# yenanjing/mmEgo

Measured on AMD Instinct MI355X. Metric: train frames/sec (Upper+Lower U+L step, B=64/GPU, T=8, 128 pts), higher is better.
Workload: dtype f32; 1 GPU; U+L step (Train_Upper + Train_Lower train_once bodies), B=64/GPU T=8 N=128, fp32, dropout live, two concurrent HIP-graph branches; global_batch=64, seq_len=8, points=128, parallelism=dp1

## Files before the change

include/mmego_hip.h:

```cpp
#ifndef MMEGO_HIP_H
#define MMEGO_HIP_H
#ifdef __cplusplus
extern "C" {
#endif

int mmego_gemm(void* stream, const float* A, long sam, long sak, const float* B, long sbk, long sbn, float* C,
               long scm, long scn, const float* bias, int M, int N, int K, int nbatch, long sAb, long sBb, long sCb,
               int relu, int accumulate, float* splitk_ws, int nsplit, long sBiasb, const float* cmul, float* asum);
typedef struct MmegoGemmDesc {
  const float* A; long sam, sak;
  const float* B; long sbk, sbn;
  float* C; long scm, scn;
  const float* bias;
  int M, N, K, nbatch;
  long sAb, sBb, sCb;
  int relu, accumulate;
  float* splitk_ws; int nsplit;
  long sBiasb;
  const float* cmul; float* asum;
} MmegoGemmDesc;
int mmego_gemm_group(void* stream, int n, const MmegoGemmDesc* descs);

int mmego_colstats_nblk(long rows);
int mmego_bn_train_stats(void* stream, const float* X, long ldx, long rows, int C, const float* gamma,
// ... 40 lines not shown

int mmego_lstm_step(void* stream, int ndir, int Bn, int H, int first, const float* hprev0, const float* hprev1,
                    long hps, const float* whh0, const float* whh1, const float* bhh0, const float* bhh1,
                    const float* xproj0, const float* xproj1, long xs, float* hout0, float* hout1, long hos, float* c0,
                    float* c1, float* gst0, float* gst1, float* cst0, float* cst1);
int mmego_lstm64_forward(void* stream, int B, int T, const float* xproj0, const float* xproj1, long xs,
                         const float* whh0, const float* whh1, const float* bhh0, const float* bhh1, const float* h0_0,
                         const float* h0_1, const float* c0_0, const float* c0_1, float* out, long os, float* hn0,
                         float* hn1, float* cn0, float* cn1,
                         float* gates0, float* gates1, float* cst0, float* cst1, float* hprev0, float* hprev1,
                         float* drop_y, float* drop_mask, float drop_p, const unsigned long long* seed_ctr, int salt);
int mmego_lstm64_backward(void* stream, int B, int T, const float* dout, long dos, const float* gates0,
                          const float* gates1, const float* cst0, const float* cst1, const float* c0_0,
                          const float* c0_1, const float* whh0, const float* whh1, float* dgates0, float* dgates1,
                          long dgs);

typedef struct MmegoLstm64Fwd {
  const float* xproj[2]; long xs;
  const float* whh[2]; const float* bhh[2]; const float* h0[2]; const float* c0[2];
  float* out; long os;
  float* hn[2]; float* cn[2];
  float* gates[2]; float* cst[2]; float* hprev[2];
  int B, T;
  float* drop_y; float* drop_mask; float drop_p; const unsigned long long* seed_ctr; unsigned salt;
} MmegoLstm64Fwd;
typedef struct MmegoLstm64Bwd {
  const float* dout; long dos;
  const float* gates[2]; const float* cst[2]; const float* c0[2]; const float* whh[2];
  float* dgates[2]; long dgs;
  int B, T;
} MmegoLstm64Bwd;
int mmego_lstm64_forward_multi(void* stream, int n, const void* descs);
int mmego_lstm64_backward_multi(void* stream, int n, const void* descs);

int mmego_cvt_bf16(void* stream, const float* X, long ldx, long rows, long cols, unsigned short* Y, long ldy);
int mmego_cvt_bf16_tm(void* stream, const float* X, long ldx, int Bn, int T, long cols, unsigned short* Y, int Bp);
int mmego_gemm_bf16(void* stream, const unsigned short* A, long lda, const unsigned short* W, long ldw, float* C,
                    long ldc, unsigned short* Cb, long ldcb, float* Cf, const float* bias, int M, int N, int K, int relu);
int mmego_lstm_step_bf16(void* stream, int ndir, int Bn, int H, int first, const unsigned short* hprev0,
                         const unsigned short* hprev1, const unsigned short* whh0, const unsigned short* whh1,
                         const float* xpf, long mt0_0, long mt0_1, float* hout0, float* hout1,
                         long hos, unsigned short* houtb0, unsigned short* houtb1, long hbs,
                         unsigned short* hfrag0, unsigned short* hfrag1, float* c0, float* c1);

int mmego_lstm_step_bf16_fused(void* stream, int ndir, int Bn, int H, int first, int nseg,
                               const unsigned short* a0_0, const unsigned short* a0_1, const unsigned short* w0_0,
                               const unsigned short* w0_1, int K0, const unsigned short* a1_0,
                               const unsigned short* a1_1, const unsigned short* w1_0, const unsigned short* w1_1,
                               int K1, const unsigned short* hprev0, const unsigned short* hprev1,
                               const unsigned short* whh0, const unsigned short* whh1, const float* bias,
                               float* hout0, float* hout1, long hos, unsigned short* hfrag0, unsigned short* hfrag1,
                               float* c0, float* c1);
int mmego_attn_pool_frag_bf16_ok(int H);
int mmego_attn_pool_frag_bf16(void* stream, const unsigned short* hf, int T, int Bp, int Bn, int H, const float* w, const float* b,
                              float* vec, float* attn);
int mmego_cvt_bf16_frag_tm(void* stream, const float* X, long ldx, int Bn, int T, int C, unsigned short* Y, int Bp);
int mmego_fc_relu_bf16_frag_tm(void* stream, const float* X, long ldx, const float* W, const float* bias, int Bn, int T, int Cin,
                               int H, unsigned short* Y, int Bp, int relu);

int mmego_lstm_cell_backward(void* stream, int ndir, int Bn, int H, const float* dout0, const float* dout1, long dos,
                             const float* dhrec0, const float* dhrec1, const float* gst0, const float* gst1,
                             const float* cst0, const float* cst1, const float* cprev0, const float* cprev1, float* dc0,
                             float* dc1, float* dgates0, float* dgates1, long dgs);
int mmego_imu_loss(void* stream, const float* R, const float* t, const float* R_gt, const float* head_gt, long F,
                   float scale, float* loss, float* dR, float* dt);
int mmego_lstm_bwd_step(void* stream, int Bn, int H, const float* dg0, const float* dg1, long dgs, const float* wT0,
// ... 238 lines not shown
```

mmego_amd/csrc/gemm.hip:

```cpp
#include <stdlib.h>

#include "common.h"
#include "../../include/mmego_hip.h"

#include "gemm_tile.h"
#include "lstm_cell.h"
#include "tile_order.h"

struct GemmP {
  const float* A;
  const float* B;
  float* C;
  const float* bias;
  long sam, sak, sbk, sbn, scm, scn;
  long sAb, sBb, sCb, sCs, sBiasb;
  int M, N, K;
  int nsplit, kchunk;
  int relu, accumulate;
  int avec, bvec;
  const float* cmul;
  float* asum;
  const float* cb_dout[2]; long cb_dos;
  const float* cb_gst[2]; const float* cb_cst[2]; const float* cb_cprev[2];
  float* cb_dc[2]; float* cb_dg[2]; long cb_dgs;
// ... 415 lines not shown
    const float bv = bias ? bias[col] : 0.0f;
#pragma unroll
    for (int i = 0; i < 2; ++i) {
#pragma unroll
      for (int reg = 0; reg < 16; ++reg) {
        int row = m0 + wm * 64 + i * 32 + (reg & 3) + 8 * (reg >> 2) + 4 * (lane >> 5);
        float v = acc[i][j][reg] + bv;
        if (relu) v = fmaxf(v, 0.0f);
        C[(long)row * ldc + col] = v;
      }
    }
  }
}

extern "C" int mmego_gemm(void* stream, const float* A, long sam, long sak, const float* B, long sbk, long sbn,
                          float* C, long scm, long scn, const float* bias, int M, int N, int K, int nbatch, long sAb,
                          long sBb, long sCb, int relu, int accumulate, float* splitk_ws, int nsplit, long sBiasb,
                          const float* cmul, float* asum) {
  MMEGO_REQUIRE(A && B && C && M > 0 && N > 0 && K > 0 && nbatch > 0 && nsplit >= 1);
  const bool defer = accumulate == 2;
  MMEGO_REQUIRE(!defer || (nsplit > 1 && nbatch == 1 && !bias && !relu));
  MMEGO_REQUIRE(!cmul || nsplit == 1);
  MMEGO_REQUIRE(relu == 0 || relu == 1 || (relu == 2 && cmul));
  MMEGO_REQUIRE(sBiasb == 0 || nsplit == 1);
  hipStream_t st = (hipStream_t)stream;
  {
    const bool a_kc = sak == 1, a_mc = sam == 1 && !a_kc;
    const bool b_kc = sbk == 1, b_mc = sbn == 1 && !b_kc;
    const long lda = a_kc ? sam : sak, ldw = b_kc ? sbn : sbk;
    const int kchunk_t = nsplit > 1 ? cdiv(cdiv(K, nsplit), 64) * 64 : K;
    constexpr long tile_min_other = GEMM_TILE_MIN_OTHER;
    const long tile_min_units = (a_kc && b_kc && nsplit == 1) ? (K <= 1024 ? 1 : 200) : tile_min_other;
    const long units64 = (long)(M / 64) * (N / 64) * nsplit * nbatch;
    const bool ok = !cmul && !asum && scn == 1 && (nbatch == 1 || ((sAb % 4) == 0 && (sBb % 4) == 0)) && (a_kc || a_mc) && (b_kc || b_mc) && (lda % 4) == 0 && (ldw % 4) == 0 &&
                    (((uintptr_t)A | (uintptr_t)B) & 15) == 0 && (M % 64) == 0 && (N % 64) == 0 &&
                    (K % 64) == 0 && units64 >= tile_min_units && (nsplit == 1 || (long)(nsplit - 1) * kchunk_t < K);
    if (ok) {
      TileP tp;
      tp.A = A; tp.W = B; tp.C = C; tp.bias = bias;
      tp.M = M; tp.N = N; tp.K = K;
      tp.lda = lda; tp.ldw = ldw; tp.ldc = scm;
      tp.relu = relu; tp.accumulate = accumulate;
      tp.nsplit = nsplit; tp.kchunk = kchunk_t; tp.ws = splitk_ws;
      tp.nbatch = nbatch; tp.sAb = sAb; tp.sWb = sBb; tp.sCb = sCb; tp.sBiasb = sBiasb;
      int rc = mmego_detail::gemm_tile_launch(st, tp, a_kc, b_kc);
      if (rc == 0 && nsplit > 1 && !defer) {
        long total = (long)nbatch * M * N;
        int blocks = (int)((total + SKR_OUT - 1) / SKR_OUT);
        hipLaunchKernelGGL(splitk_reduce_kernel, dim3(blocks), dim3(256), 0, st, splitk_ws, C, bias, nsplit, nbatch, M, N, scm, scn,
                           sCb, relu, accumulate, (const float*)nullptr, (float*)nullptr);
        MMEGO_LAUNCH_CHECK();
      }
      if (rc != -2) return rc;
    }
  }
  const bool fast = !cmul && !asum && nbatch == 1 && nsplit == 1 && !accumulate && sak == 1 && sbk == 1 && scn == 1 && (M % 128) == 0 &&
                    (N % 128) == 0 && (K % 16) == 0 && (sam % 4) == 0 && (sbn % 4) == 0 &&
                    (((uintptr_t)A | (uintptr_t)B) & 15) == 0;
  if (fast) {
    dim3 grid((M / 128) * (N / 128));
    hipLaunchKernelGGL(gemm128_nt_kernel, grid, dim3(256), 0, st, A, B, C, bias, M, N, K, sam, sbn, scm, relu);
    MMEGO_LAUNCH_CHECK();
    return MMEGO_OK;
  }
  GemmP p;
  p.A = A; p.B = B; p.bias = bias;
  p.sam = sam; p.sak = sak; p.sbk = sbk; p.sbn = sbn;
  p.sAb = sAb; p.sBb = sBb; p.sBiasb = sBiasb;
  p.M = M; p.N = N; p.K = K;
  p.nsplit = nsplit;
  p.relu = relu; p.accumulate = accumulate;
  p.cmul = cmul;
  p.asum = asum;
  p.cb_dg[0] = p.cb_dg[1] = nullptr;
  if (nsplit > 1) {
    MMEGO_REQUIRE(splitk_ws != nullptr);
    int kc = cdiv(K, nsplit);
// ... 131 lines not shown
```

mmego_amd/csrc/gemm_tile.h:

```cpp
#pragma once
#include <hip/hip_runtime.h>

struct TileP {
  const float* A;
  const float* W;
  float* C;
  const float* bias;
  int M, N, K;
  long lda, ldw, ldc;
  int relu, accumulate;
  int nsplit, kchunk;
  float* ws;
  int nbatch;
  long sAb, sWb, sCb, sBiasb;
};

namespace mmego_detail {
int gemm_tile_launch(hipStream_t st, const TileP& p, bool a_kc, bool b_kc);
}
```

mmego_amd/csrc/gemm_tile.hip:

```cpp
#include <stdlib.h>

#include "common.h"
#include "gemm_tile.h"
#include "lds_dma.h"
#include "tile_order.h"

#define TLD_MAX 68

template <int BM, int BN, int WAVES_M, int WAVES_N, bool A_KC, bool B_KC, int KCH>
__device__ __forceinline__ void gemm_tile_body(const TileP& p, int m0, int n0, int sb, float* smem, int sid) {
  const int split = sb % p.nsplit, batch = sb / p.nsplit;
  static_assert(WAVES_M * WAVES_N == 4, "4 waves");
  static_assert(KCH == 64 || KCH == 32, "k per staged chunk");
  constexpr int TLD = KCH + 4;
  constexpr int WM = BM / WAVES_M, WN = BN / WAVES_N;
  constexpr int TM = WM / 32, TN = WN / 32;
  constexpr int AV = BM * KCH / 1024, BV = BN * KCH / 1024;
  constexpr int LPR = KCH / 4, RPP = 256 / LPR;
  constexpr int ALD = BM + 4, BLD = BN + 4;
  constexpr int ARP = 1024 / BM, BRP = 1024 / BN;
  float* As = smem;
  float* Bs = smem + BM * TLD;
  const int tid = threadIdx.x, lane = tid & 63, wave = tid >> 6;
  const int wm = wave % WAVES_M, wn = wave / WAVES_M;
// ... 262 lines not shown
      }
      if (kb == 3) {
        asm volatile("s_waitcnt vmcnt(0) lgkmcnt(0)" ::: "memory");
        __builtin_amdgcn_s_barrier();
        if (kt + 2 < nk) GTB_DMA(kt + 2, kt & 1)
      }
#pragma unroll
      for (int c = 0; c < 4; ++c)
#pragma unroll
        for (int i = 0; i < 5; ++i)
#pragma unroll
          for (int j = 0; j < 2; ++j) acc[i][j] = __builtin_amdgcn_mfma_f32_32x32x2f32(a[i][c], b[j][c], acc[i][j], 0, 0, 0);
    }
  }
#endif
#undef GTB_DMA
  const bool slabs = p.nsplit > 1;
  float* C = slabs ? p.ws + (long)blockIdx.y * p.M * p.N : p.C + (long)batch * p.sCb;
  const long ldc = slabs ? (long)p.N : p.ldc;
#pragma unroll
  for (int j = 0; j < 2; ++j) {
    const int col = n0 + wn * 64 + j * 32 + r;
    const float bv = (p.bias && !slabs) ? p.bias[(long)batch * p.sBiasb + col] : 0.0f;
#pragma unroll
    for (int i = 0; i < 5; ++i) {
      float* cp = C + (long)(m0 + wm * 160 + i * 32 + 4 * h) * ldc + col;
#pragma unroll
      for (int reg = 0; reg < 16; ++reg)
        if (!(GTB_EXP & 4) || acc[i][j][reg] == 12345.f) cp[(long)((reg & 3) + 8 * (reg >> 2)) * ldc] = acc[i][j][reg] + bv;
    }
  }
}

namespace mmego_detail {

constexpr int GT_KCH = 32;

template <int BM, int BN, bool A_KC, bool B_KC, int KCH>
static int launch_plain_k(hipStream_t st, const TileP& p) {
  const size_t lds = (size_t)((BM + BN) * (KCH + 4)) * sizeof(float);
  if (int e = mmego_allow_lds<gemm_tile_kernel<BM, BN, 2, 2, A_KC, B_KC, KCH>>(lds)) return e;
  const unsigned units = (unsigned)((p.M / BM) * (p.N / BN) * p.nsplit * p.nbatch);
  hipLaunchKernelGGL((gemm_tile_kernel<BM, BN, 2, 2, A_KC, B_KC, KCH>), dim3(units), dim3(256), lds, st, p);
  hipError_t e = hipGetLastError();
  return e == hipSuccess ? 0 : (int)e;
}

template <int BM, int BN, bool A_KC, bool B_KC>
static int launch_plain(hipStream_t st, const TileP& p) { return launch_plain_k<BM, BN, A_KC, B_KC, GT_KCH>(st, p); }

template <bool A_KC, bool B_KC>
static int launch_layout(hipStream_t st, const TileP& p) {
  if (A_KC && B_KC) {
    static const bool big = !(getenv("MMEGO_GEMM_BIG") && atoi(getenv("MMEGO_GEMM_BIG")) == 0);
    const long tiles = (long)(p.M / 320) * (p.N / 256) * p.nbatch;
    const bool slab_ok = p.nsplit == 1 ? !p.accumulate
                                       : (p.accumulate == 2 && p.nbatch == 1 && p.ws && !p.bias && (p.kchunk % 32) == 0 && p.kchunk >= 64 &&
                                          (long)(p.nsplit - 1) * p.kchunk < p.K && (p.K - (long)(p.nsplit - 1) * p.kchunk) >= 64);
    const long units = tiles * p.nsplit;
    if (big && (p.M % 320) == 0 && (p.N % 256) == 0 && (p.K % 32) == 0 && p.K >= 64 && slab_ok && !p.relu &&
        units >= 256 && (units % 256) == 0 && tiles < (1L << 30) && (p.lda % 4) == 0 && (p.ldw % 4) == 0 && (p.sAb % 4) == 0 && (p.sWb % 4) == 0 &&
        ((((uintptr_t)p.A) | ((uintptr_t)p.W)) & 15) == 0) {
      constexpr int lds = 2 * (320 + 256) * 32 * (int)sizeof(float);
      if (int e = mmego_allow_lds<gemm_tile_big_kernel<0>>(lds)) return e;
      TileBigArgs g = {p.M / 320, p.N / 256};
      hipLaunchKernelGGL((gemm_tile_big_kernel<0>), dim3((unsigned)tiles, (unsigned)p.nsplit), dim3(512), lds, st, p, g);
      hipError_t e = hipGetLastError();
      return e == hipSuccess ? 0 : (int)e;
    }
  }
  const long units128 = (long)(p.M / 128) * (p.N / 128) * p.nsplit * p.nbatch;
  const bool big_ok = (p.M % 128) == 0 && (p.N % 128) == 0 && units128 >= 192;
  if (big_ok) {
    static const int slots = getenv("MMEGO_GEMM_SLOTS") ? atoi(getenv("MMEGO_GEMM_SLOTS")) : 512;
    const int units = (int)units128;
    if (units > slots && p.K > 128) {
      const int rest = units % slots;
      const bool halves = rest > 0 && rest <= slots / 2;
      const int nfull = halves ? units - rest : units, nhalf = halves ? 2 * rest : 0;
      const size_t lds = slots <= 256 ? 84 * 1024 : (size_t)(256 * (GT_KCH + 4)) * sizeof(float);
      if (int e = mmego_allow_lds<gemm_tile_persistent_kernel<A_KC, B_KC, GT_KCH>>(lds)) return e;
      hipLaunchKernelGGL((gemm_tile_persistent_kernel<A_KC, B_KC, GT_KCH>), dim3(slots), dim3(256), lds, st, p, nfull, nhalf, 1);
      hipError_t e = hipGetLastError();
      return e == hipSuccess ? 0 : (int)e;
    }
    return launch_plain<128, 128, A_KC, B_KC>(st, p);
  }
  return launch_plain<64, 64, A_KC, B_KC>(st, p);
}

int gemm_tile_launch(hipStream_t st, const TileP& p, bool a_kc, bool b_kc) {
  if ((p.K % 64) != 0 || (p.M % 64) != 0 || (p.N % 64) != 0 || p.nsplit < 1 || p.nbatch < 1) return -2;
  if (p.nsplit > 1 && ((p.kchunk % 64) != 0 || p.ws == nullptr)) return -2;
  if (a_kc && b_kc) return launch_layout<true, true>(st, p);
  if (a_kc) return launch_layout<true, false>(st, p);
  if (b_kc) return launch_layout<false, true>(st, p);
  return launch_layout<false, false>(st, p);
}

}
```

mmego_amd/csrc/lstm.hip:

```cpp
#include "common.h"
#include "lstm_cell.h"
#include <stddef.h>
#include "../../include/mmego_hip.h"

struct Lstm64P {
  const float* xproj[2]; long xs;
  const float* whh[2];
  const float* bhh[2];
  const float* h0[2]; const float* c0[2];
  float* out; long os;
  float* hn[2]; float* cn[2];
  float* gates[2]; float* cst[2]; float* hprev[2];
  int B, T;
  float* drop_y; float* drop_mask; float drop_p; const unsigned long long* seed_ctr; unsigned salt;
};


#define L64_LDS_BARRIER() asm volatile("s_waitcnt lgkmcnt(0)\n\ts_barrier" ::: "memory")

#define WLD 272

typedef const float __attribute__((address_space(1)))* l64_gcptr;
typedef float __attribute__((address_space(1)))* l64_gptr;
typedef f32x4 __attribute__((address_space(1)))* l64_gptr4;
// ... 104 lines not shown
          const float mk = dropout_keep(dkey, (unsigned)off, p.drop_p) ? keep_scale : 0.f;
          p.drop_mask[off] = mk;
          p.drop_y[off] = hn * mk;
        }
        if (stash) {
          *(l64_gptr4)gq[reg] = (f32x4){u.i, u.f, u.g, u.o};
          *cq[reg] = cn;
        }
      }
      oq[reg] += ostep;
      if (stash) { gq[reg] += gstep; cq[reg] += cstep; }
    }
    __builtin_amdgcn_sched_barrier(0);
#pragma unroll
    for (int g = 0; g < 4; ++g)
#pragma unroll
      for (int reg = 0; reg < 4; ++reg) xp[g][reg] = xpn[g][reg];
    L64_LDS_BARRIER();
  }
#undef L64_LOAD_XP
#pragma unroll
  for (int reg = 0; reg < 4; ++reg) {
    int row = r0 + fq * 4 + reg;
    if (row < B) {
      if (p.hn[d]) p.hn[d][row * 64 + j] = hreg[reg];
      if (p.cn[d]) p.cn[d][row * 64 + j] = creg[reg];
    }
  }
}

template <bool FULL, bool STASH, bool DROP>
__global__ __launch_bounds__(256) void lstm64_fwd_kernel(Lstm64P p) { lstm64_fwd_body<FULL, STASH, DROP>(p); }

#define L64_MAX_MULTI 4
static_assert(sizeof(Lstm64P) == sizeof(MmegoLstm64Fwd) && offsetof(Lstm64P, seed_ctr) == offsetof(MmegoLstm64Fwd, seed_ctr) &&
              offsetof(Lstm64P, B) == offsetof(MmegoLstm64Fwd, B), "MmegoLstm64Fwd is Lstm64P");
struct Lstm64Multi { Lstm64P p[L64_MAX_MULTI]; };
template <bool FULL, bool STASH, bool DROP>
__global__ __launch_bounds__(256) void lstm64_fwd_multi_kernel(Lstm64Multi m) { lstm64_fwd_body<FULL, STASH, DROP>(m.p[blockIdx.z]); }

extern "C" int mmego_lstm64_forward(void* stream, int B, int T, const float* xproj0, const float* xproj1, long xs,
                                    const float* whh0, const float* whh1, const float* bhh0, const float* bhh1,
                                    const float* h0_0, const float* h0_1, const float* c0_0, const float* c0_1, float* out,
                                    long os, float* hn0, float* hn1,
                                    float* cn0, float* cn1, float* gates0, float* gates1, float* cst0, float* cst1,
                                    float* hprev0, float* hprev1, float* drop_y, float* drop_mask, float drop_p,
                                    const unsigned long long* seed_ctr, int salt) {
  MMEGO_REQUIRE((drop_mask == nullptr) == (drop_y == nullptr));
  MMEGO_REQUIRE(!drop_mask || (seed_ctr && drop_p > 0.f && drop_p < 1.f && (long)B * T * os < (1L << 32)));
  MMEGO_REQUIRE(B > 0 && T > 0 && xproj0 && xproj1 && whh0 && whh1 && out);
  MMEGO_REQUIRE((((uintptr_t)whh0 | (uintptr_t)whh1) & 15) == 0);
  MMEGO_REQUIRE((gates0 == nullptr) == (cst0 == nullptr) && (gates1 == nullptr) == (cst1 == nullptr));
  Lstm64P p;
  p.xproj[0] = xproj0; p.xproj[1] = xproj1; p.xs = xs;
  p.whh[0] = whh0; p.whh[1] = whh1;
  p.bhh[0] = bhh0; p.bhh[1] = bhh1;
  p.h0[0] = h0_0; p.h0[1] = h0_1; p.c0[0] = c0_0; p.c0[1] = c0_1;
  p.out = out; p.os = os;
  p.hn[0] = hn0; p.hn[1] = hn1; p.cn[0] = cn0; p.cn[1] = cn1;
  p.gates[0] = gates0; p.gates[1] = gates1; p.cst[0] = cst0; p.cst[1] = cst1;
  p.hprev[0] = hprev0; p.hprev[1] = hprev1;
  p.B = B; p.T = T;
  p.drop_y = drop_y; p.drop_mask = drop_mask; p.drop_p = drop_p; p.seed_ctr = seed_ctr; p.salt = (unsigned)salt;
  size_t lds = (size_t)(64 * 16) * sizeof(float);
  const bool full = B % 16 == 0, st_ = gates0 != nullptr, dr = drop_mask != nullptr;
  MMEGO_REQUIRE((hprev0 != nullptr) == st_ && (hprev1 != nullptr) == st_ && (gates1 != nullptr) == st_);
#define L64_FWD_LAUNCH(F_, S_, D_)                                                                                    \
  do {                                                                                                                \
    if (int e = mmego_allow_lds<lstm64_fwd_kernel<F_, S_, D_>>(lds)) return e;                                        \
    hipLaunchKernelGGL((lstm64_fwd_kernel<F_, S_, D_>), dim3(cdiv(B, 16), 2), dim3(256), lds, (hipStream_t)stream, p); \
  } while (0)
  if (full) {
    if (st_ && dr) L64_FWD_LAUNCH(true, true, true);
    else if (st_) L64_FWD_LAUNCH(true, true, false);
    else if (dr) L64_FWD_LAUNCH(true, false, true);
    else L64_FWD_LAUNCH(true, false, false);
  } else {
    if (st_ && dr) L64_FWD_LAUNCH(false, true, true);
    else if (st_) L64_FWD_LAUNCH(false, true, false);
    else if (dr) L64_FWD_LAUNCH(false, false, true);
    else L64_FWD_LAUNCH(false, false, false);
  }
#undef L64_FWD_LAUNCH
  MMEGO_LAUNCH_CHECK();
  return MMEGO_OK;
}

struct Lstm64BwdP {
  const float* dout; long dos;
  const float* gates[2]; const float* cst[2]; const float* c0[2];
  const float* whh[2];
  float* dgates[2]; long dgs;
  int B, T;
};


template <bool FULL>
__device__ __forceinline__ void lstm64_bwd_body(const Lstm64BwdP& p) {
  extern __shared__ __attribute__((aligned(16))) float smem[];
  float* dgs = smem;
  const int tid = threadIdx.x, lane = tid & 63, wave = tid >> 6;
// ... 69 lines not shown
#pragma unroll
      for (int g = 0; g < 4; ++g) dgs[(g * 64 + j) * 16 + fq * 4 + reg] = dg4[g][reg];
      ccur[reg] = gin[reg][5];
    }
    L64_LDS_BARRIER();
    f32x4 a0 = {0.f, 0.f, 0.f, 0.f}, a1 = {0.f, 0.f, 0.f, 0.f}, a2 = {0.f, 0.f, 0.f, 0.f}, a3 = {0.f, 0.f, 0.f, 0.f};
#pragma unroll
    for (int nb = 0; nb < 64; nb += 16) {
      float dk[16];
#pragma unroll
      for (int u = 0; u < 16; ++u) dk[u] = dgs[((nb + u) * 4 + fq) * 16 + fr];
      __builtin_amdgcn_sched_barrier(0);
#pragma unroll
      for (int u = 0; u < 16; u += 4) {
        a0 = __builtin_amdgcn_mfma_f32_16x16x4f32(dk[u], wreg[nb + u], a0, 0, 0, 0);
        a1 = __builtin_amdgcn_mfma_f32_16x16x4f32(dk[u + 1], wreg[nb + u + 1], a1, 0, 0, 0);
        a2 = __builtin_amdgcn_mfma_f32_16x16x4f32(dk[u + 2], wreg[nb + u + 2], a2, 0, 0, 0);
        a3 = __builtin_amdgcn_mfma_f32_16x16x4f32(dk[u + 3], wreg[nb + u + 3], a3, 0, 0, 0);
      }
    }
    dhrec = (a0 + a1) + (a2 + a3);
    __builtin_amdgcn_sched_barrier(0);
#pragma unroll
    for (int reg = 0; reg < 4; ++reg)
#pragma unroll
      for (int q = 0; q < 6; ++q) gin[reg][q] = gnx[reg][q];
    L64_LDS_BARRIER();
  }
#undef L64_LOAD_BWD
}

template <bool FULL>
__global__ __launch_bounds__(256) void lstm64_bwd_kernel(Lstm64BwdP p) { lstm64_bwd_body<FULL>(p); }
static_assert(sizeof(Lstm64BwdP) == sizeof(MmegoLstm64Bwd) && offsetof(Lstm64BwdP, dgs) == offsetof(MmegoLstm64Bwd, dgs), "MmegoLstm64Bwd is Lstm64BwdP");
struct Lstm64BwdMulti { Lstm64BwdP p[L64_MAX_MULTI]; };
template <bool FULL>
__global__ __launch_bounds__(256) void lstm64_bwd_multi_kernel(Lstm64BwdMulti m) { lstm64_bwd_body<FULL>(m.p[blockIdx.z]); }

extern "C" int mmego_lstm64_backward(void* stream, int B, int T, const float* dout, long dos, const float* gates0,
                                     const float* gates1, const float* cst0, const float* cst1, const float* c0_0,
                                     const float* c0_1, const float* whh0, const float* whh1, float* dgates0,
                                     float* dgates1, long dgs) {
  MMEGO_REQUIRE(B > 0 && T > 0 && dout && gates0 && gates1 && cst0 && cst1 && whh0 && whh1 && dgates0 && dgates1);
  MMEGO_REQUIRE((((uintptr_t)whh0 | (uintptr_t)whh1) & 15) == 0);
  Lstm64BwdP p;
  p.dout = dout; p.dos = dos;
  p.gates[0] = gates0; p.gates[1] = gates1; p.cst[0] = cst0; p.cst[1] = cst1;
  p.c0[0] = c0_0; p.c0[1] = c0_1;
  p.whh[0] = whh0; p.whh[1] = whh1;
  p.dgates[0] = dgates0; p.dgates[1] = dgates1; p.dgs = dgs;
  p.B = B; p.T = T;
  const size_t lds = (size_t)(256 * 16) * sizeof(float);
  if (B % 16 == 0) hipLaunchKernelGGL(lstm64_bwd_kernel<true>, dim3(cdiv(B, 16), 2), dim3(256), lds, (hipStream_t)stream, p);
  else hipLaunchKernelGGL(lstm64_bwd_kernel<false>, dim3(cdiv(B, 16), 2), dim3(256), lds, (hipStream_t)stream, p);
  MMEGO_LAUNCH_CHECK();
  return MMEGO_OK;
}

extern "C" int mmego_lstm64_forward_multi(void* stream, int n, const void* descs) {
  MMEGO_REQUIRE(descs && n >= 1 && n <= L64_MAX_MULTI);
  const Lstm64P* h = static_cast<const Lstm64P*>(descs);
  Lstm64Multi m;
  const int B = h[0].B, T = h[0].T;
  const bool st_ = h[0].gates[0] != nullptr, dr = h[0].drop_mask != nullptr;
  for (int i = 0; i < n; ++i) {
    const Lstm64P& p = h[i];
    MMEGO_REQUIRE(p.B == B && p.T == T && B > 0 && T > 0 && p.xproj[0] && p.xproj[1] && p.whh[0] && p.whh[1] && p.out);
    MMEGO_REQUIRE((((uintptr_t)p.whh[0] | (uintptr_t)p.whh[1]) & 15) == 0);
    MMEGO_REQUIRE((p.drop_mask == nullptr) == (p.drop_y == nullptr) && (p.drop_mask != nullptr) == dr);
    MMEGO_REQUIRE(!p.drop_mask || (p.seed_ctr && p.drop_p > 0.f && p.drop_p < 1.f && (long)B * T * p.os < (1L << 32)));
    MMEGO_REQUIRE((p.gates[0] != nullptr) == st_ && (p.gates[1] != nullptr) == st_ && (p.cst[0] != nullptr) == st_ && (p.cst[1] != nullptr) == st_ &&
                  (p.hprev[0] != nullptr) == st_ && (p.hprev[1] != nullptr) == st_);
    m.p[i] = p;
  }
  for (int i = n; i < L64_MAX_MULTI; ++i) m.p[i] = h[0];
  const size_t lds = (size_t)(64 * 16) * sizeof(float);
  const bool full = B % 16 == 0;
#define L64_FWDM_LAUNCH(F_, S_, D_) hipLaunchKernelGGL((lstm64_fwd_multi_kernel<F_, S_, D_>), dim3(cdiv(B, 16), 2, n), dim3(256), lds, (hipStream_t)stream, m)
  if (full) {
    if (st_ && dr) L64_FWDM_LAUNCH(true, true, true);
    else if (st_) L64_FWDM_LAUNCH(true, true, false);
    else if (dr) L64_FWDM_LAUNCH(true, false, true);
    else L64_FWDM_LAUNCH(true, false, false);
  } else {
    if (st_ && dr) L64_FWDM_LAUNCH(false, true, true);
    else if (st_) L64_FWDM_LAUNCH(false, true, false);
    else if (dr) L64_FWDM_LAUNCH(false, false, true);
    else L64_FWDM_LAUNCH(false, false, false);
  }
#undef L64_FWDM_LAUNCH
  MMEGO_LAUNCH_CHECK();
  return MMEGO_OK;
}

extern "C" int mmego_lstm64_backward_multi(void* stream, int n, const void* descs) {
  MMEGO_REQUIRE(descs && n >= 1 && n <= L64_MAX_MULTI);
  const Lstm64BwdP* h = static_cast<const Lstm64BwdP*>(descs);
  Lstm64BwdMulti m;
  const int B = h[0].B, T = h[0].T;
  for (int i = 0; i < n; ++i) {
    const Lstm64BwdP& p = h[i];
    MMEGO_REQUIRE(p.B == B && p.T == T && B > 0 && T > 0 && p.dout && p.gates[0] && p.gates[1] && p.cst[0] && p.cst[1] && p.whh[0] && p.whh[1] &&
                  p.dgates[0] && p.dgates[1]);
    MMEGO_REQUIRE((((uintptr_t)p.whh[0] | (uintptr_t)p.whh[1]) & 15) == 0);
    m.p[i] = p;
  }
  for (int i = n; i < L64_MAX_MULTI; ++i) m.p[i] = h[0];
  const size_t lds = (size_t)(256 * 16) * sizeof(float);
  if (B % 16 == 0) hipLaunchKernelGGL(lstm64_bwd_multi_kernel<true>, dim3(cdiv(B, 16), 2, n), dim3(256), lds, (hipStream_t)stream, m);
  else hipLaunchKernelGGL(lstm64_bwd_multi_kernel<false>, dim3(cdiv(B, 16), 2, n), dim3(256), lds, (hipStream_t)stream, m);
  MMEGO_LAUNCH_CHECK();
  return MMEGO_OK;
}
```

mmego_amd/hip.py:

```python
import ctypes
import os
import re

import torch

_HERE = os.path.dirname(os.path.abspath(__file__))
HEADER = os.path.join(os.path.dirname(_HERE), "include", "mmego_hip.h")
LIBPATH = os.environ.get("MMEGO_HIP_LIB") or os.path.join(_HERE, "lib", "libmmego_hip.so")

_CT = {"int": ctypes.c_int, "long": ctypes.c_long, "float": ctypes.c_float, "double": ctypes.c_double}


def parse_header(path=HEADER):
    text = open(path).read()
    text = re.sub(r"/\*.*?\*/", " ", text, flags=re.S)
    protos = {}
    for m in re.finditer(r"\bint\s+(mmego_\w+)\s*\(([^)]*)\)\s*;", text):
        args = []
        for a in m.group(2).split(","):
            a = " ".join(a.split())
            if not a or a == "void":
                continue
            name = re.search(r"(\w+)$", a).group(1)
            typ = a[: -len(name)].strip()
# ... 161 lines not shown
def _gemm_out_extents(args):
    out = []
    M, N, nb = int(args[10]), int(args[11]), max(1, int(args[13]))
    c = _ptr_of(args[6])
    if c is not None:
        span = (M - 1) * abs(int(args[7])) + (N - 1) * abs(int(args[8])) + 1
        for b in range(nb):
            lo = c + 4 * b * int(args[16])
            out.append((lo, lo + 4 * span))
    s = _ptr_of(args[23])
    if s is not None:
        out.append((s, s + 4 * M * nb))
    return out


def call(name, *args):
    if _gemm_rec is not None and name != "gemm_group":
        for a in args:
            p = _ptr_of(a)
            if p is not None and any(lo <= p < hi for lo, hi in _gemm_rec_outs):
                raise RuntimeError("gemm_group: mmego_%s takes the output of a product that is still deferred inside this context "
                                   "(only independent leaves may be grouped)" % name)
        if name == "gemm":
            _gemm_rec_outs.extend(_gemm_out_extents(args))
            _gemm_rec.append(args)
            return
    _launch(name, *args)


def graph_dA_nblk(G):
    return lib().mmego_graph_dA_nblk(G)


def colstats_nblk(rows):
    return lib().mmego_colstats_nblk(rows)
```

Before: 105,100 frames/s.

## Add 4-row LSTM64 recurrent kernels and a wide 64x128 GEMM tile path

Result: faster. 107,400 frames/s, median of 6 (+2.2%).

```diff
diff --git a/include/mmego_hip.h b/include/mmego_hip.h
--- a/include/mmego_hip.h
+++ b/include/mmego_hip.h
@@ -96,6 +96,7 @@
 } MmegoLstm64Bwd;
 int mmego_lstm64_forward_multi(void* stream, int n, const void* descs);
 int mmego_lstm64_backward_multi(void* stream, int n, const void* descs);
+int mmego_lstm64_rows_per_workgroup(int B, int T);
 
 int mmego_cvt_bf16(void* stream, const float* X, long ldx, long rows, long cols, unsigned short* Y, long ldy);
 int mmego_cvt_bf16_tm(void* stream, const float* X, long ldx, int Bn, int T, long cols, unsigned short* Y, int Bp);
diff --git a/mmego_amd/csrc/gemm.hip b/mmego_amd/csrc/gemm.hip
--- a/mmego_amd/csrc/gemm.hip
+++ b/mmego_amd/csrc/gemm.hip
@@ -471,17 +471,19 @@
     constexpr long tile_min_other = GEMM_TILE_MIN_OTHER;
     const long tile_min_units = (a_kc && b_kc && nsplit == 1) ? (K <= 1024 ? 1 : 200) : tile_min_other;
     const long units64 = (long)(M / 64) * (N / 64) * nsplit * nbatch;
-    const bool ok = !cmul && !asum && scn == 1 && (nbatch == 1 || ((sAb % 4) == 0 && (sBb % 4) == 0)) && (a_kc || a_mc) && (b_kc || b_mc) && (lda % 4) == 0 && (ldw % 4) == 0 &&
-                    (((uintptr_t)A | (uintptr_t)B) & 15) == 0 && (M % 64) == 0 && (N % 64) == 0 &&
-                    (K % 64) == 0 && units64 >= tile_min_units && (nsplit == 1 || (long)(nsplit - 1) * kchunk_t < K);
+    TileP tp;
+    tp.A = A; tp.W = B; tp.C = C; tp.bias = bias;
+    tp.M = M; tp.N = N; tp.K = K;
+    tp.lda = lda; tp.ldw = ldw; tp.ldc = scm;
+    tp.relu = relu; tp.accumulate = accumulate;
+    tp.nsplit = nsplit; tp.kchunk = kchunk_t; tp.ws = splitk_ws;
+    tp.nbatch = nbatch; tp.sAb = sAb; tp.sWb = sBb; tp.sCb = sCb; tp.sBiasb = sBiasb;
+    const bool wide = !cmul && !asum && scn == 1 && a_kc && b_kc && gemm_tile_wide_fits(tp);
+    const bool ok = wide ||
+                    (!cmul && !asum && scn == 1 && (nbatch == 1 || ((sAb % 4) == 0 && (sBb % 4) == 0)) && (a_kc || a_mc) && (b_kc || b_mc) && (lda % 4) == 0 && (ldw % 4) == 0 &&
+                     (((uintptr_t)A | (uintptr_t)B) & 15) == 0 && (M % 64) == 0 && (N % 64) == 0 &&
+                     (K % 64) == 0 && units64 >= tile_min_units && (nsplit == 1 || (long)(nsplit - 1) * kchunk_t < K));
     if (ok) {
-      TileP tp;
-      tp.A = A; tp.W = B; tp.C = C; tp.bias = bias;
-      tp.M = M; tp.N = N; tp.K = K;
-      tp.lda = lda; tp.ldw = ldw; tp.ldc = scm;
-      tp.relu = relu; tp.accumulate = accumulate;
-      tp.nsplit = nsplit; tp.kchunk = kchunk_t; tp.ws = splitk_ws;
-      tp.nbatch = nbatch; tp.sAb = sAb; tp.sWb = sBb; tp.sCb = sCb; tp.sBiasb = sBiasb;
       int rc = mmego_detail::gemm_tile_launch(st, tp, a_kc, b_kc);
       if (rc == 0 && nsplit > 1 && !defer) {
         long total = (long)nbatch * M * N;
diff --git a/mmego_amd/csrc/gemm_tile.h b/mmego_amd/csrc/gemm_tile.h
--- a/mmego_amd/csrc/gemm_tile.h
+++ b/mmego_amd/csrc/gemm_tile.h
@@ -1,5 +1,6 @@
 #pragma once
 #include <hip/hip_runtime.h>
+#include <stdint.h>
 
 struct TileP {
   const float* A;
@@ -15,6 +16,13 @@
   long sAb, sWb, sCb, sBiasb;
 };
 
+inline bool gemm_tile_wide_fits(const TileP& p) {
+  return p.M <= 1024 && p.N >= 2048 && (p.M % 64) == 0 && (p.N % 128) == 0 && p.K >= 32 && (p.K % 32) == 0 && p.nsplit == 1 && p.nbatch >= 1 &&
+         (p.accumulate == 0 || p.accumulate == 1) && (p.relu == 0 || p.relu == 1) && (p.lda % 4) == 0 && (p.ldw % 4) == 0 &&
+         (p.nbatch == 1 || ((p.sAb % 4) == 0 && (p.sWb % 4) == 0)) && (long)(p.M / 64) * (p.N / 128) * p.nbatch < (1L << 30) &&
+         ((((uintptr_t)p.A) | ((uintptr_t)p.W)) & 15) == 0;
+}
+
 namespace mmego_detail {
 int gemm_tile_launch(hipStream_t st, const TileP& p, bool a_kc, bool b_kc);
 }
diff --git a/mmego_amd/csrc/gemm_tile.hip b/mmego_amd/csrc/gemm_tile.hip
--- a/mmego_amd/csrc/gemm_tile.hip
+++ b/mmego_amd/csrc/gemm_tile.hip
@@ -318,6 +318,118 @@
   }
 }
 
+template <int DUMMY>
+__global__ __launch_bounds__(256) void gemm_tile_wide_kernel(TileP p, TileBigArgs g) {
+  constexpr int BM = 64, BN = 128, KCH = 32, ROWS = BM + BN, STAGE = ROWS * KCH, NT = ROWS / 8 / 4;
+  extern __shared__ __attribute__((aligned(16))) float smem[];
+  const int tid = threadIdx.x, lane = tid & 63;
+  const int w = __builtin_amdgcn_readfirstlane(tid >> 6);
+  const int wm = w & 1, wn = w >> 1;
+  const TileMN t = panel_walk_or_row_major(blockIdx.x, gridDim.x, g.tiles_m, g.tiles_n);
+  const int batch = t.m / g.tiles_m;
+  const int m0 = (t.m - batch * g.tiles_m) * BM, n0 = t.n * BN;
+  const float* Ab = p.A + (long)batch * p.sAb + (long)m0 * p.lda;
+  const float* Wb = p.W + (long)batch * p.sWb + (long)n0 * p.ldw;
+  const float* gp[NT];
+#pragma unroll
+  for (int j = 0; j < NT; ++j) {
+    const int i = w + 4 * j;
+    const bool isw = i >= BM / 8;
+    const int row = (isw ? i - BM / 8 : i) * 8 + (lane >> 3);
+    const int piece = (lane & 7) ^ ((row >> 1) & 7);
+    gp[j] = (isw ? Wb + (long)row * p.ldw : Ab + (long)row * p.lda) + 4 * piece;
+  }
+#define GTW_DMA1(kt, stage, j) GLDS16(gp[j] + (long)(kt) * KCH, smem + (stage) * STAGE + (w + 4 * (j)) * 8 * KCH)
+#define GTW_DMA(kt, stage)                                                                        \
+  {                                                                                               \
+    _Pragma("unroll") for (int j = 0; j < NT; ++j) GTW_DMA1(kt, stage, j);                        \
+  }
+#define GTW_SB() __builtin_amdgcn_sched_barrier(0)
+#define GTW_USE(x) asm volatile("" ::"v"(x))
+  const int nk = p.K / KCH;
+  const int r = lane & 31, h = lane >> 5, key = (r >> 1) & 7;
+  int off[4];
+#pragma unroll
+  for (int kb = 0; kb < 4; ++kb) off[kb] = r * KCH + 4 * ((2 * kb + h) ^ key);
+  const int aoff = wm * 32 * KCH, boff = (BM + wn * 64) * KCH;
+  f32x16 acc[2];
+#pragma unroll
+  for (int j = 0; j < 2; ++j) acc[j] = (f32x16){0};
+  GTW_DMA(0, 0)
+  if (nk > 1) GTW_DMA(1, 1)
+  if (nk > 1) wait_vmcnt<NT>();
+  else wait_vmcnt<0>();
+  __builtin_amdgcn_s_barrier();
+  f32x4 a[2], b[2][2];
+  a[0] = *reinterpret_cast<const f32x4*>(smem + aoff + off[0]);
+#pragma unroll
+  for (int j = 0; j < 2; ++j) b[0][j] = *reinterpret_cast<const f32x4*>(smem + boff + j * 32 * KCH + off[0]);
+  int cur = 0, nxt = 1, thr = 2;
+  for (int kt = 0; kt < nk; ++kt) {
+    const float* Sc = smem + cur * STAGE;
+    const float* Sn = smem + nxt * STAGE;
+    const bool ahead = kt + 2 < nk;
+#pragma unroll
+    for (int kb = 0; kb < 4; ++kb) {
+      GTW_USE(a[kb & 1]); GTW_USE(b[kb & 1][0]); GTW_USE(b[kb & 1][1]);
+      GTW_SB();
+      if (kb < 3) {
+        a[(kb + 1) & 1] = *reinterpret_cast<const f32x4*>(Sc + aoff + off[kb + 1]);
+#pragma unroll
+        for (int j = 0; j < 2; ++j) b[(kb + 1) & 1][j] = *reinterpret_cast<const f32x4*>(Sc + boff + j * 32 * KCH + off[kb + 1]);
+      } else if (kt + 1 < nk) {
+        if (kt + 2 < nk) wait_vmcnt<NT>();
+        else wait_vmcnt<0>();
+        wait_lgkmcnt0();
+        __builtin_amdgcn_s_barrier();
+        a[0] = *reinterpret_cast<const f32x4*>(Sn + aoff + off[0]);
+#pragma unroll
+        for (int j = 0; j < 2; ++j) b[0][j] = *reinterpret_cast<const f32x4*>(Sn + boff + j * 32 * KCH + off[0]);
+      }
+      GTW_SB();
+#pragma unroll
+      for (int c = 0; c < 4; ++c) {
+#pragma unroll
+        for (int j = 0; j < 2; ++j) acc[j] = __builtin_amdgcn_mfma_f32_32x32x2f32(a[kb & 1][c], b[kb & 1][j][c], acc[j], 0, 0, 0);
+        if (kb < 3 && c < 2) {
+          GTW_SB();
+          if (ahead) GTW_DMA1(kt + 2, thr, 2 * kb + c);
+          GTW_SB();
+        }
+      }
+      GTW_SB();
+    }
+    const int t_ = cur;
+    cur = nxt; nxt = thr; thr = t_;
+  }
+#undef GTW_DMA
+#undef GTW_DMA1
+#undef GTW_SB
+#undef GTW_USE
+  float* C = p.C + (long)batch * p.sCb;
+  const bool relu = p.relu, accumulate = p.accumulate;
+#pragma unroll
+  for (int j = 0; j < 2; ++j) {
+    const int col = n0 + wn * 64 + j * 32 + r;
+    const float bv = p.bias ? p.bias[(long)batch * p.sBiasb + col] : 0.0f;
+    float* cp = C + (long)(m0 + wm * 32 + 4 * h) * p.ldc + col;
+    float old[16];
+    if (accumulate) {
+#pragma unroll
+      for (int reg = 0; reg < 16; ++reg) old[reg] = cp[(long)((reg & 3) + 8 * (reg >> 2)) * p.ldc];
+#pragma unroll
+      for (int reg = 0; reg < 16; ++reg) asm volatile("" : "+v"(old[reg]));
+    }
+#pragma unroll
+    for (int reg = 0; reg < 16; ++reg) {
+      float v = acc[j][reg] + bv;
+      if (relu) v = fmaxf(v, 0.0f);
+      if (accumulate) v += old[reg];
+      cp[(long)((reg & 3) + 8 * (reg >> 2)) * p.ldc] = v;
+    }
+  }
+}
+
 namespace mmego_detail {
 
 constexpr int GT_KCH = 32;
@@ -355,6 +467,14 @@
       return e == hipSuccess ? 0 : (int)e;
     }
   }
+  if (A_KC && B_KC && gemm_tile_wide_fits(p)) {
+    constexpr int lds = 3 * (64 + 128) * 32 * (int)sizeof(float);
+    if (int e = mmego_allow_lds<gemm_tile_wide_kernel<0>>(lds)) return e;
+    TileBigArgs g = {p.M / 64, p.N / 128};
+    hipLaunchKernelGGL((gemm_tile_wide_kernel<0>), dim3((unsigned)((long)g.tiles_m * g.tiles_n * p.nbatch)), dim3(256), lds, st, p, g);
+    hipError_t e = hipGetLastError();
+    return e == hipSuccess ? 0 : (int)e;
+  }
   const long units128 = (long)(p.M / 128) * (p.N / 128) * p.nsplit * p.nbatch;
   const bool big_ok = (p.M % 128) == 0 && (p.N % 128) == 0 && units128 >= 192;
   if (big_ok) {
@@ -376,6 +496,7 @@
 }
 
 int gemm_tile_launch(hipStream_t st, const TileP& p, bool a_kc, bool b_kc) {
+  if (a_kc && b_kc && gemm_tile_wide_fits(p)) return launch_layout<true, true>(st, p);
   if ((p.K % 64) != 0 || (p.M % 64) != 0 || (p.N % 64) != 0 || p.nsplit < 1 || p.nbatch < 1) return -2;
   if (p.nsplit > 1 && ((p.kchunk % 64) != 0 || p.ws == nullptr)) return -2;
   if (a_kc && b_kc) return launch_layout<true, true>(st, p);
diff --git a/mmego_amd/csrc/lstm.hip b/mmego_amd/csrc/lstm.hip
--- a/mmego_amd/csrc/lstm.hip
+++ b/mmego_amd/csrc/lstm.hip
@@ -160,12 +160,157 @@
 template <bool FULL, bool STASH, bool DROP>
 __global__ __launch_bounds__(256) void lstm64_fwd_kernel(Lstm64P p) { lstm64_fwd_body<FULL, STASH, DROP>(p); }
 
+#define H4LD 68
+template <int CTRL>
+__device__ __forceinline__ float l64_quad_perm(float v) {
+  return __builtin_bit_cast(float, __builtin_amdgcn_update_dpp(0, __builtin_bit_cast(int, v), CTRL, 0xF, 0xF, true));
+}
+#define L64_QP_XOR1 0xB1
+#define L64_QP_XOR2 0x4E
+
+template <bool FULL, bool STASH, bool DROP>
+__device__ __forceinline__ void lstm64_fwd4_body(const Lstm64P& p) {
+  extern __shared__ __attribute__((aligned(16))) float smem[];
+  const int tid = threadIdx.x, lane = tid & 63, wave = tid >> 6;
+  const int d = blockIdx.y, r0 = blockIdx.x * 4;
+  const int B = p.B, T = p.T;
+  const int q = lane & 3;
+  const int j = wave * 16 + (lane >> 2);
+  const int row = r0 + q;
+  const bool live = FULL || row < B;
+  float bh[4];
+#pragma unroll
+  for (int g = 0; g < 4; ++g) bh[g] = p.bhh[d] ? p.bhh[d][g * 64 + j] : 0.f;
+  float creg = (row < B && p.c0[d]) ? p.c0[d][row * 64 + j] : 0.f;
+  float hreg = (row < B && p.h0[d]) ? p.h0[d][row * 64 + j] : 0.f;
+  smem[q * H4LD + j] = hreg;
+  __syncthreads();
+  float wreg[64];
+  {
+    const float* wrow = p.whh[d] + (q * 64 + j) * 64;
+#pragma unroll
+    for (int m = 0; m < 16; ++m) {
+      const f32x4 v = *reinterpret_cast<const f32x4*>(wrow + 4 * m);
+      wreg[4 * m + 0] = v.x; wreg[4 * m + 1] = v.y; wreg[4 * m + 2] = v.z; wreg[4 * m + 3] = v.w;
+    }
+  }
+  float xp[4], xpn[4];
+  constexpr bool stash = STASH, keep_h = STASH, drop = DROP;
+  const unsigned dkey = drop ? dropout_key(p.seed_ctr[0], p.salt) : 0u;
+  const float keep_scale = drop ? 1.0f / (1.0f - p.drop_p) : 1.0f;
+  const int t_first = d == 0 ? 0 : T - 1;
+  const long dir = d == 0 ? 1 : -1;
+  const long rt = (long)(live ? row : 0) * T + t_first;
+  const long tr = (long)t_first * B + (live ? row : 0);
+  l64_gcptr xq = (l64_gcptr)(p.xproj[d] + rt * p.xs + j);
+  l64_gptr oq = (l64_gptr)(p.out + rt * p.os + d * 64 + j);
+  l64_gptr hq = keep_h ? (l64_gptr)(p.hprev[d] + rt * 64 + j) : (l64_gptr)nullptr;
+  l64_gptr gq = stash ? (l64_gptr)(p.gates[d] + tr * 256 + 4 * j) : (l64_gptr)nullptr;
+  l64_gptr cq = stash ? (l64_gptr)(p.cst[d] + tr * 64 + j) : (l64_gptr)nullptr;
+  const long xstep = dir * p.xs, ostep = dir * p.os, hstep = dir * 64, gstep = dir * (long)B * 256, cstep = dir * (long)B * 64;
+#define L64_LOAD_XP4(DST)                                                                  \
+  do {                                                                                     \
+    _Pragma("unroll") for (int g = 0; g < 4; ++g) DST[g] = live ? xq[g * 64] : 0.f;        \
+    xq += xstep;                                                                           \
+  } while (0)
+  L64_LOAD_XP4(xp);
+  int cur = 0;
+  for (int s = 0; s < T; ++s) {
+    if (s + 1 >= T) xq -= xstep;
+    L64_LOAD_XP4(xpn);
+    if (keep_h) {
+      if (live) *hq = hreg;
+      hq += hstep;
+    }
+    const float* hb = smem + cur + q * H4LD;
+    f32x4 hk[16];
+#pragma unroll
+    for (int mm = 0; mm < 16; ++mm) {
+      const int m = (mm & 3) * 4 + (mm >> 2);
+      hk[m] = *reinterpret_cast<const f32x4*>(hb + 4 * m);
+    }
+    __builtin_amdgcn_sched_barrier(0);
+    f32x4 acc = {0.f, 0.f, 0.f, 0.f};
+#pragma unroll
+    for (int k4 = 0; k4 < 16; ++k4)
+#pragma unroll
+      for (int fq = 0; fq < 4; ++fq) {
+        const int k = 16 * fq + k4;
+        acc = __builtin_amdgcn_mfma_f32_4x4x1f32(hk[k >> 2][k & 3], wreg[k], acc, 0, 0, 0);
+      }
+    float z[4];
+    {
+      const bool b0 = q & 1, b1 = q & 2;
+      float w[4];
+#pragma unroll
+      for (int pr = 0; pr < 2; ++pr) {
+        const float recv = l64_quad_perm<L64_QP_XOR1>(b0 ? acc[2 * pr] : acc[2 * pr + 1]);
+        w[2 * pr] = b0 ? recv : acc[2 * pr];
+        w[2 * pr + 1] = b0 ? acc[2 * pr + 1] : recv;
+      }
+#pragma unroll
+      for (int e = 0; e < 2; ++e) {
+        const float recv = l64_quad_perm<L64_QP_XOR2>(b1 ? w[e] : w[e + 2]);
+        z[e] = b1 ? recv : w[e];
+        z[e + 2] = b1 ? w[e + 2] : recv;
+      }
+    }
+    const LstmCell u = lstm_cell_fwd(z[0] + (xp[0] + bh[0]), z[1] + (xp[1] + bh[1]), z[2] + (xp[2] + bh[2]), z[3] + (xp[3] + bh[3]), creg);
+    const float cn = u.c, hn = u.h;
+    creg = cn;
+    hreg = hn;
+    cur ^= 4 * H4LD;
+    smem[cur + q * H4LD + j] = hn;
+    if (live) {
+      *oq = hn;
+      if (drop) {
+        const long off = oq - (l64_gptr)p.out;
+        const float mk = dropout_keep(dkey, (unsigned)off, p.drop_p) ? keep_scale : 0.f;
+        p.drop_mask[off] = mk;
+        p.drop_y[off] = hn * mk;
+      }
+      if (stash) {
+        *(l64_gptr4)gq = (f32x4){u.i, u.f, u.g, u.o};
+        *cq = cn;
+      }
+    }
+    oq += ostep;
+    if (stash) { gq += gstep; cq += cstep; }
+    __builtin_amdgcn_sched_barrier(0);
+#pragma unroll
+    for (int g = 0; g < 4; ++g) xp[g] = xpn[g];
+    L64_LDS_BARRIER();
+  }
+#undef L64_LOAD_XP4
+  if (row < B) {
+    if (p.hn[d]) p.hn[d][row * 64 + j] = hreg;
+    if (p.cn[d]) p.cn[d][row * 64 + j] = creg;
+  }
+}
+
+template <bool FULL, bool STASH, bool DROP>
+__global__ __launch_bounds__(256) void lstm64_fwd4_kernel(Lstm64P p) { lstm64_fwd4_body<FULL, STASH, DROP>(p); }
+
 #define L64_MAX_MULTI 4
 static_assert(sizeof(Lstm64P) == sizeof(MmegoLstm64Fwd) && offsetof(Lstm64P, seed_ctr) == offsetof(MmegoLstm64Fwd, seed_ctr) &&
               offsetof(Lstm64P, B) == offsetof(MmegoLstm64Fwd, B), "MmegoLstm64Fwd is Lstm64P");
 struct Lstm64Multi { Lstm64P p[L64_MAX_MULTI]; };
 template <bool FULL, bool STASH, bool DROP>
 __global__ __launch_bounds__(256) void lstm64_fwd_multi_kernel(Lstm64Multi m) { lstm64_fwd_body<FULL, STASH, DROP>(m.p[blockIdx.z]); }
+template <bool FULL, bool STASH, bool DROP>
+__global__ __launch_bounds__(256) void lstm64_fwd4_multi_kernel(Lstm64Multi m) { lstm64_fwd4_body<FULL, STASH, DROP>(m.p[blockIdx.z]); }
+
+#ifndef L64_FORCE_ROWS
+#define L64_FORCE_ROWS 0
+#endif
+#define L64_ROWS4_MAX_B 256
+#define L64_LDS4_FWD ((size_t)(2 * 4 * H4LD) * sizeof(float))
+#define L64_LDS4_BWD ((size_t)(4 * DG4LD + 4 * 4 * PS4LD) * sizeof(float))
+extern "C" int mmego_lstm64_rows_per_workgroup(int B, int T) {
+  (void)T;
+  if (L64_FORCE_ROWS) return L64_FORCE_ROWS;
+  return B <= L64_ROWS4_MAX_B ? 4 : 16;
+}
 
 extern "C" int mmego_lstm64_forward(void* stream, int B, int T, const float* xproj0, const float* xproj1, long xs,
                                     const float* whh0, const float* whh1, const float* bhh0, const float* bhh1,
@@ -191,10 +336,15 @@
   p.B = B; p.T = T;
   p.drop_y = drop_y; p.drop_mask = drop_mask; p.drop_p = drop_p; p.seed_ctr = seed_ctr; p.salt = (unsigned)salt;
   size_t lds = (size_t)(64 * 16) * sizeof(float);
-  const bool full = B % 16 == 0, st_ = gates0 != nullptr, dr = drop_mask != nullptr;
+  const bool four = mmego_lstm64_rows_per_workgroup(B, T) == 4;
+  const bool full = B % (four ? 4 : 16) == 0, st_ = gates0 != nullptr, dr = drop_mask != nullptr;
   MMEGO_REQUIRE((hprev0 != nullptr) == st_ && (hprev1 != nullptr) == st_ && (gates1 != nullptr) == st_);
 #define L64_FWD_LAUNCH(F_, S_, D_)                                                                                    \
   do {                                                                                                                \
+    if (four) {                                                                                                       \
+      hipLaunchKernelGGL((lstm64_fwd4_kernel<F_, S_, D_>), dim3(cdiv(B, 4), 2), dim3(256), L64_LDS4_FWD, (hipStream_t)stream, p); \
+      break;                                                                                                          \
+    }                                                                                                                 \
     if (int e = mmego_allow_lds<lstm64_fwd_kernel<F_, S_, D_>>(lds)) return e;                                        \
     hipLaunchKernelGGL((lstm64_fwd_kernel<F_, S_, D_>), dim3(cdiv(B, 16), 2), dim3(256), lds, (hipStream_t)stream, p); \
   } while (0)
@@ -330,10 +480,107 @@
 
 template <bool FULL>
 __global__ __launch_bounds__(256) void lstm64_bwd_kernel(Lstm64BwdP p) { lstm64_bwd_body<FULL>(p); }
+
+#define DG4LD 260
+#define PS4LD 80
+template <bool FULL>
+__device__ __forceinline__ void lstm64_bwd4_body(const Lstm64BwdP& p) {
+  extern __shared__ __attribute__((aligned(16))) float smem[];
+  float* dgs = smem;
+  float* ps = smem + 4 * DG4LD;
+  const int tid = threadIdx.x, lane = tid & 63, wave = tid >> 6;
+  const int d = blockIdx.y, r0 = blockIdx.x * 4;
+  const int B = p.B, T = p.T;
+  const int q = lane & 3, j = wave * 16 + (lane >> 2);
+  const int row = r0 + q;
+  const bool live = FULL || row < B;
+  float wreg[64];
+  {
+    const float* W = p.whh[d] + lane;
+#pragma unroll
+    for (int m = 0; m < 16; ++m)
+#pragma unroll
+      for (int f = 0; f < 4; ++f) wreg[4 * m + f] = W[(4 * (wave + 4 * m) + f) * 64];
+  }
+  float dcreg = 0.f, dhrec = 0.f;
+  float gin[6], gnx[6];
+  float ccur;
+  const l64_gcptr g_gates = (l64_gcptr)p.gates[d], g_dout = (l64_gcptr)p.dout, g_cst = (l64_gcptr)p.cst[d];
+  const bool has_c0 = p.c0[d] != nullptr;
+  const l64_gcptr g_c0 = has_c0 ? (l64_gcptr)p.c0[d] : g_cst;
+#define L64_LOAD_BWD4(DST, step)                                                                                 \
+  do {                                                                                                           \
+    const int tq_ = d == 0 ? (step) : T - 1 - (step);                                                            \
+    const int tp_ = d == 0 ? tq_ - 1 : tq_ + 1;                                                                  \
+    if (live) {                                                                                                  \
+      const f32x4 gv_ = *(l64_gcptr4)(g_gates + ((long)tq_ * B + row) * 256 + 4 * j);                            \
+      DST[0] = g_dout[((long)row * T + tq_) * p.dos + d * 64 + j];                                               \
+      DST[1] = gv_.x; DST[2] = gv_.y; DST[3] = gv_.z; DST[4] = gv_.w;                                            \
+      const l64_gcptr cp_ = ((step) > 0) ? g_cst + ((long)tp_ * B + row) * 64 + j : g_c0 + (long)row * 64 + j;   \
+      const float cv_ = *cp_;                                                                                    \
+      DST[5] = ((step) > 0 || has_c0) ? cv_ : 0.f;                                                               \
+    } else {                                                                                                     \
+      _Pragma("unroll") for (int x_ = 0; x_ < 6; ++x_) DST[x_] = 0.f;                                            \
+    }                                                                                                            \
+  } while (0)
+  L64_LOAD_BWD4(gin, T - 1);
+  {
+    const int tl = d == 0 ? T - 1 : 0;
+    ccur = live ? g_cst[((long)tl * B + row) * 64 + j] : 0.f;
+  }
+  for (int s = T - 1; s >= 0; --s) {
+    const int tt = d == 0 ? s : T - 1 - s;
+    const int sn = s > 0 ? s - 1 : 0;
+    L64_LOAD_BWD4(gnx, sn);
+    float dg4[4];
+    if (live) {
+      const float dh = gin[0] + dhrec;
+      const LstmCellGrad o = lstm_cell_bwd(gin[1], gin[2], gin[3], gin[4], fast_tanh(ccur), gin[5], dcreg, dh);
+      dg4[0] = o.di; dg4[1] = o.df; dg4[2] = o.dg; dg4[3] = o.dout;
+      dcreg = o.dcprev;
+      l64_gptr dst = (l64_gptr)p.dgates[d] + ((long)row * T + tt) * p.dgs + j;
+#pragma unroll
+      for (int g = 0; g < 4; ++g) dst[g * 64] = dg4[g];
+    } else {
+#pragma unroll
+      for (int g = 0; g < 4; ++g) dg4[g] = 0.f;
+    }
+#pragma unroll
+    for (int g = 0; g < 4; ++g) dgs[q * DG4LD + g * 64 + j] = dg4[g];
+    ccur = gin[5];
+    L64_LDS_BARRIER();
+    f32x4 dk[16];
+#pragma unroll
+    for (int m = 0; m < 16; ++m) dk[m] = *reinterpret_cast<const f32x4*>(dgs + q * DG4LD + 4 * (wave + 4 * m));
+    __builtin_amdgcn_sched_barrier(0);
+    f32x4 acc = {0.f, 0.f, 0.f, 0.f};
+#pragma unroll
+    for (int m = 0; m < 16; ++m)
+#pragma unroll
+      for (int f = 0; f < 4; ++f) acc = __builtin_amdgcn_mfma_f32_4x4x1f32(dk[m][f], wreg[4 * m + f], acc, 0, 0, 0);
+#pragma unroll
+    for (int i = 0; i < 4; ++i) ps[(wave * 4 + i) * PS4LD + lane] = acc[i];
+    L64_LDS_BARRIER();
+    {
+      const float a0 = ps[(0 * 4 + q) * PS4LD + j], a1 = ps[(1 * 4 + q) * PS4LD + j], a2 = ps[(2 * 4 + q) * PS4LD + j],
+                  a3 = ps[(3 * 4 + q) * PS4LD + j];
+      dhrec = (a0 + a1) + (a2 + a3);
+    }
+    __builtin_amdgcn_sched_barrier(0);
+#pragma unroll
+    for (int x = 0; x < 6; ++x) gin[x] = gnx[x];
+  }
+#undef L64_LOAD_BWD4
+}
+
+template <bool FULL>
+__global__ __launch_bounds__(256) void lstm64_bwd4_kernel(Lstm64BwdP p) { lstm64_bwd4_body<FULL>(p); }
 static_assert(sizeof(Lstm64BwdP) == sizeof(MmegoLstm64Bwd) && offsetof(Lstm64BwdP, dgs) == offsetof(MmegoLstm64Bwd, dgs), "MmegoLstm64Bwd is Lstm64BwdP");
 struct Lstm64BwdMulti { Lstm64BwdP p[L64_MAX_MULTI]; };
 template <bool FULL>
 __global__ __launch_bounds__(256) void lstm64_bwd_multi_kernel(Lstm64BwdMulti m) { lstm64_bwd_body<FULL>(m.p[blockIdx.z]); }
+template <bool FULL>
+__global__ __launch_bounds__(256) void lstm64_bwd4_multi_kernel(Lstm64BwdMulti m) { lstm64_bwd4_body<FULL>(m.p[blockIdx.z]); }
 
 extern "C" int mmego_lstm64_backward(void* stream, int B, int T, const float* dout, long dos, const float* gates0,
                                      const float* gates1, const float* cst0, const float* cst1, const float* c0_0,
@@ -349,7 +596,10 @@
   p.dgates[0] = dgates0; p.dgates[1] = dgates1; p.dgs = dgs;
   p.B = B; p.T = T;
   const size_t lds = (size_t)(256 * 16) * sizeof(float);
-  if (B % 16 == 0) hipLaunchKernelGGL(lstm64_bwd_kernel<true>, dim3(cdiv(B, 16), 2), dim3(256), lds, (hipStream_t)stream, p);
+  if (mmego_lstm64_rows_per_workgroup(B, T) == 4) {
+    if (B % 4 == 0) hipLaunchKernelGGL(lstm64_bwd4_kernel<true>, dim3(cdiv(B, 4), 2), dim3(256), L64_LDS4_BWD, (hipStream_t)stream, p);
+    else hipLaunchKernelGGL(lstm64_bwd4_kernel<false>, dim3(cdiv(B, 4), 2), dim3(256), L64_LDS4_BWD, (hipStream_t)stream, p);
+  } else if (B % 16 == 0) hipLaunchKernelGGL(lstm64_bwd_kernel<true>, dim3(cdiv(B, 16), 2), dim3(256), lds, (hipStream_t)stream, p);
   else hipLaunchKernelGGL(lstm64_bwd_kernel<false>, dim3(cdiv(B, 16), 2), dim3(256), lds, (hipStream_t)stream, p);
   MMEGO_LAUNCH_CHECK();
   return MMEGO_OK;
@@ -373,8 +623,13 @@
   }
   for (int i = n; i < L64_MAX_MULTI; ++i) m.p[i] = h[0];
   const size_t lds = (size_t)(64 * 16) * sizeof(float);
-  const bool full = B % 16 == 0;
-#define L64_FWDM_LAUNCH(F_, S_, D_) hipLaunchKernelGGL((lstm64_fwd_multi_kernel<F_, S_, D_>), dim3(cdiv(B, 16), 2, n), dim3(256), lds, (hipStream_t)stream, m)
+  const bool four = mmego_lstm64_rows_per_workgroup(B, T) == 4;
+  const bool full = B % (four ? 4 : 16) == 0;
+#define L64_FWDM_LAUNCH(F_, S_, D_)                                                                                                        \
+  do {                                                                                                                                     \
+    if (four) hipLaunchKernelGGL((lstm64_fwd4_multi_kernel<F_, S_, D_>), dim3(cdiv(B, 4), 2, n), dim3(256), L64_LDS4_FWD, (hipStream_t)stream, m); \
+    else hipLaunchKernelGGL((lstm64_fwd_multi_kernel<F_, S_, D_>), dim3(cdiv(B, 16), 2, n), dim3(256), lds, (hipStream_t)stream, m);      \
+  } while (0)
   if (full) {
     if (st_ && dr) L64_FWDM_LAUNCH(true, true, true);
     else if (st_) L64_FWDM_LAUNCH(true, true, false);
@@ -405,7 +660,10 @@
   }
   for (int i = n; i < L64_MAX_MULTI; ++i) m.p[i] = h[0];
   const size_t lds = (size_t)(256 * 16) * sizeof(float);
-  if (B % 16 == 0) hipLaunchKernelGGL(lstm64_bwd_multi_kernel<true>, dim3(cdiv(B, 16), 2, n), dim3(256), lds, (hipStream_t)stream, m);
+  if (mmego_lstm64_rows_per_workgroup(B, T) == 4) {
+    if (B % 4 == 0) hipLaunchKernelGGL(lstm64_bwd4_multi_kernel<true>, dim3(cdiv(B, 4), 2, n), dim3(256), L64_LDS4_BWD, (hipStream_t)stream, m);
+    else hipLaunchKernelGGL(lstm64_bwd4_multi_kernel<false>, dim3(cdiv(B, 4), 2, n), dim3(256), L64_LDS4_BWD, (hipStream_t)stream, m);
+  } else if (B % 16 == 0) hipLaunchKernelGGL(lstm64_bwd_multi_kernel<true>, dim3(cdiv(B, 16), 2, n), dim3(256), lds, (hipStream_t)stream, m);
   else hipLaunchKernelGGL(lstm64_bwd_multi_kernel<false>, dim3(cdiv(B, 16), 2, n), dim3(256), lds, (hipStream_t)stream, m);
   MMEGO_LAUNCH_CHECK();
   return MMEGO_OK;
diff --git a/mmego_amd/hip.py b/mmego_amd/hip.py
--- a/mmego_amd/hip.py
+++ b/mmego_amd/hip.py
@@ -217,5 +217,9 @@
     return lib().mmego_graph_dA_nblk(G)
 
 
+def lstm64_rows_per_workgroup(B, T):
+    return lib().mmego_lstm64_rows_per_workgroup(B, T)
+
+
 def colstats_nblk(rows):
     return lib().mmego_colstats_nblk(rows)
```
